# kdavila/lecturemath

Measured on AMD Instinct MI355X. Metric: frames/sec end-to-end binarize+CC+group @1080p, higher is better.
Workload: dtype u8

## Files before the change

lecturemath_amd/csrc/lm_api.hip:

```cpp
#include "lm_common.h"
#include "lm_stream.h"

#include <stdarg.h>
#include <stdlib.h>
#include <stdio.h>
#include <string.h>

#include "../../include/lecturemath_amd.h"

#include "lm_cc_kernels.hip"
#include "lm_match_kernels.hip"
#include "lm_match_batch.hip"
#include "lm_group.hip"
#include "lm_fcn.hip"
#include "lm_fcn2.hip"

static thread_local char g_err[512] = "";

void lm_set_error(const char* fmt, ...)
{
    va_list ap;
    va_start(ap, fmt);
    vsnprintf(g_err, sizeof(g_err), fmt, ap);
    va_end(ap);
// ... 492 lines not shown
    bool ok = hipMemcpy(c->stage_i32, labels, px * sizeof(int32_t), hipMemcpyHostToDevice) == hipSuccess;
    if (ok && ages) ok = hipMemcpy(c->stage_f32, ages, px * sizeof(float), hipMemcpyHostToDevice) == hipSuccess;
    if (ok) {
        const float* d_ages = ages ? c->stage_f32 : (const float*)nullptr;
        hipLaunchKernelGGL(lm_k_ab_init, dim3(lm_blocks(n, 256)), dim3(256), 0, (hipStream_t)0, mny, mxy, mnx, mxx, cnt, ageb, last_px, last_neg,
                           width, height, n);
        hipLaunchKernelGGL(lm_k_ab_scan, dim3(lm_blocks((long long)px, 256)), dim3(256), 0, (hipStream_t)0, c->stage_i32, d_ages, width, height, n,
                           mny, mxy, mnx, mxx, cnt, last_px, last_neg);
        hipLaunchKernelGGL(lm_k_ab_age, dim3(lm_blocks((long long)px, 256)), dim3(256), 0, (hipStream_t)0, c->stage_i32, d_ages, width, height, n,
                           last_neg, ageb);
        hipLaunchKernelGGL(lm_k_ab_finish, dim3(lm_blocks(n, 256)), dim3(256), 0, (hipStream_t)0, ageb, last_px, last_neg, d_ages, agef, n);
        const size_t nb = (size_t)n * sizeof(int32_t);
        ok = hipMemcpy(out_mins_y, mny, nb, hipMemcpyDeviceToHost) == hipSuccess &&
             hipMemcpy(out_maxs_y, mxy, nb, hipMemcpyDeviceToHost) == hipSuccess &&
             hipMemcpy(out_mins_x, mnx, nb, hipMemcpyDeviceToHost) == hipSuccess &&
             hipMemcpy(out_maxs_x, mxx, nb, hipMemcpyDeviceToHost) == hipSuccess &&
             hipMemcpy(out_counts, cnt, nb, hipMemcpyDeviceToHost) == hipSuccess &&
             hipMemcpy(output_age, agef, nb, hipMemcpyDeviceToHost) == hipSuccess;
    }
    if (!ok) lm_set_error("CC_AgeBoundaries: device copy/launch failed");
    (void)hipFree(d_out);
    return 0;
}

extern "C" void lm_stream_destroy(LmStream* s)
{
    if (!s) return;
    void* ptrs[] = {s->cc, s->assign, s->frame_cc_off, s->crop, s->chash, s->active_cc, s->active_box, s->active_last, s->active, s->counters, s->best,
                    s->batch_cc_base, s->batch_word_base};
    for (void* p : ptrs)
        if (p) (void)hipFree(p);
    if (s->mb) {
        LmMatchBatch* m = s->mb;
        void* mp[] = {m->nt_cnt, m->nt_src, m->tlast, m->tcur[0], m->tcur[1], m->ftile_all, m->nt_foff, m->nt_list, m->cls, m->troot, m->rootpos, m->ftile, m->s_prefix, m->tcount[0], m->tcount[1], m->toff[0], m->toff[1], m->pairs[0], m->pairs[1], m->pair_u[0],
                      m->pair_u[1], m->sidx, m->s_list, m->s_box, m->newpos, m->n_src, m->ttab, m->tkey, m->twin, m->big[0], m->big[1], m->n_big};
        for (void* p : mp)
            if (p) (void)hipFree(p);
        delete m;
    }
    if (s->twin_stream) (void)hipStreamDestroy((hipStream_t)s->twin_stream);
    for (int i = 0; i < s->n_run_events; i++) (void)hipEventDestroy(s->run_events[i]);
    free(s->run_events);
    if (s->rd_scratch) (void)hipFree(s->rd_scratch);
    if (s->garena) (void)hipFree(s->garena);
    if (s->gpin) (void)hipHostFree(s->gpin);
    delete s;
}

extern "C" int lm_stream_set_min_pixels(LmStream* s, int min_pixels)
{
    if (!s || min_pixels < 0) { lm_set_error("lm_stream_set_min_pixels: bad arguments"); return LM_ERR_ARG; }
    s->min_pixels = min_pixels;
    return LM_OK;
}

extern "C" int lm_stream_reset(LmStream* s, void* stream)
{
    if (!s) { lm_set_error("lm_stream_reset: null stream"); return LM_ERR_ARG; }
    LM_HIP(hipMemsetAsync(s->counters, 0, sizeof(LmCounters), (hipStream_t)stream));
    LM_HIP(hipMemsetAsync(s->best, 0xff, (size_t)s->ctx->g.cap * sizeof(unsigned long long), (hipStream_t)stream));
    LM_HIP(hipMemsetAsync(s->frame_cc_off, 0, sizeof(long long), (hipStream_t)stream));
    LM_HIP(hipMemsetAsync(s->chash, 0, (size_t)s->cap_cc * sizeof(uint32_t), (hipStream_t)stream));
    if (s->mb) LM_HIP(hipMemsetAsync(s->mb->ttab, 0xff, (size_t)LM_MB_TTAB * sizeof(unsigned long long), (hipStream_t)stream));
    s->frames_pushed = 0;
    s->frames_matched = 0;
    s->tempo_B = 0;
    return LM_OK;
// ... 6 lines not shown
        lm_set_error("lm_stream_create: bad arguments");
        return nullptr;
    }
    LmStream* s = new LmStream();
    memset(s, 0, sizeof(*s));
    s->ctx = ctx;
    s->cap_frames = max_frames;
    s->cap_cc = max_ccs;
    s->cap_words = (unsigned long long)max_crop_words;
    s->cap_uniq = max_uniques;
    s->min_recall = min_recall;
    s->min_precision = min_precision;
    s->max_gap = max_gap;
    s->min_pixels = min_pixels;
    int rc = LM_OK;
    rc |= lm_alloc(&s->cc, (size_t)max_ccs);
    rc |= lm_alloc(&s->assign, (size_t)max_ccs);
    rc |= lm_alloc(&s->frame_cc_off, (size_t)max_frames + 1);
    rc |= lm_alloc(&s->crop, (size_t)max_crop_words);
    rc |= lm_alloc(&s->chash, (size_t)max_ccs);
    rc |= lm_alloc(&s->active_cc, (size_t)max_uniques);
    rc |= lm_alloc(&s->active_box, (size_t)max_uniques);
    rc |= lm_alloc(&s->active_last, (size_t)max_uniques);
    rc |= lm_alloc(&s->active, (size_t)max_uniques);
    rc |= lm_alloc(&s->best, (size_t)ctx->g.cap);
    rc |= lm_alloc(&s->counters, (size_t)1);
    rc |= lm_alloc(&s->batch_cc_base, (size_t)ctx->max_batch);
    rc |= lm_alloc(&s->batch_word_base, (size_t)ctx->max_batch);
    {
        LmMatchBatch* m = new LmMatchBatch();
        memset(m, 0, sizeof(*m));
        s->mb = m;
        m->cap_tiles = (int)(max_ccs / LM_MB_TILE) + max_frames + 2;
        long long cp = 16 * (long long)max_ccs;
        if (cp < (1 << 16)) cp = 1 << 16;
        if (cp > (1 << 23)) cp = 1 << 23;
        m->cap_pairs = (uint32_t)cp;
        rc |= lm_alloc(&m->ftile, (size_t)max_frames + 2);
        rc |= lm_alloc(&m->s_prefix, (size_t)max_frames + 2);
        rc |= lm_alloc(&m->ftile_all, (size_t)max_frames + 2);
        rc |= lm_alloc(&m->nt_foff, (size_t)max_frames + 2);
        rc |= lm_alloc(&m->nt_list, (size_t)max_ccs);
        rc |= lm_alloc(&m->cls, (size_t)max_ccs);
        rc |= lm_alloc(&m->troot, (size_t)max_ccs);
        rc |= lm_alloc(&m->rootpos, (size_t)max_ccs);
        rc |= lm_alloc(&m->nt_cnt, (size_t)LM_MB_MAX_FRAMES);
        rc |= lm_alloc(&m->nt_src, (size_t)max_ccs);
        rc |= lm_alloc(&m->tlast, (size_t)max_ccs);
        for (int k = 0; k < 2; k++) {
            rc |= lm_alloc(&m->tcount[k], (size_t)m->cap_tiles + 1);
            rc |= lm_alloc(&m->toff[k], (size_t)m->cap_tiles + 1);
            rc |= lm_alloc(&m->tcur[k], ((size_t)m->cap_tiles + 1) * LM_MB_JY);
            rc |= lm_alloc(&m->pairs[k], (size_t)m->cap_pairs);
            rc |= lm_alloc(&m->pair_u[k], (size_t)m->cap_pairs);
        }
        rc |= lm_alloc(&m->sidx, (size_t)max_ccs);
        rc |= lm_alloc(&m->s_list, (size_t)max_ccs);
        rc |= lm_alloc(&m->s_box, (size_t)max_ccs);
        rc |= lm_alloc(&m->newpos, (size_t)max_ccs);
        rc |= lm_alloc(&m->n_src, (size_t)1);
        rc |= lm_alloc(&m->ttab, (size_t)LM_MB_TTAB);
        rc |= lm_alloc(&m->tkey, (size_t)max_ccs);
        rc |= lm_alloc(&m->twin, (size_t)max_ccs);
        m->cap_big = 1u << 16;
        rc |= lm_alloc(&m->big[0], (size_t)m->cap_big);
        rc |= lm_alloc(&m->big[1], (size_t)m->cap_big);
        rc |= lm_alloc(&m->n_big, (size_t)2);
#if !LM_HIP_EMULATED
        if (rc == LM_OK &&
            hipFuncSetAttribute((const void*)lm_k_mb_resolve, hipFuncAttributeMaxDynamicSharedMemorySize, (int)LM_MB_RESOLVE_SMEM) != hipSuccess)
            rc = LM_ERR_HIP;
#endif
        const char* e = getenv("LM_MATCH_PER_FRAME");
        s->match_per_frame = (e && atoi(e) == 1) ? 1 : 0;
    }
    if (rc == LM_OK && hipMemset(s->mb->twin, 0, (size_t)max_ccs) != hipSuccess) rc = LM_ERR_HIP;
    if (rc == LM_OK) rc = lm_stream_reset(s, nullptr);
    if (rc == LM_OK && hipStreamSynchronize(nullptr) != hipSuccess) rc = LM_ERR_HIP;
    if (rc != LM_OK) {
        lm_stream_destroy(s);
        return nullptr;
    }
    return s;
}

static void lm_launch_match(LmStream* s, int f, hipStream_t st)
{
    hipLaunchKernelGGL(lm_k_match, LM_HIP_EMULATED ? dim3(2, 2) : dim3(16, 64), dim3(256), 0, st, s->cc, s->crop, s->frame_cc_off, f,
                       s->active_box, s->active_last, s->active_cc, s->counters, s->best, s->min_recall, s->min_precision, s->max_gap);
    hipLaunchKernelGGL(lm_k_update, dim3(1), dim3(1024), 0, st, s->cc, s->frame_cc_off, f, s->active, s->active_cc, s->active_box,
                       s->active_last, s->counters, s->assign, s->best, s->max_gap, s->cap_uniq, (f & 15) == 15 ? 1 : 0);
}

static void lm_flush_tempo(LmStream* s, hipStream_t st)
{
    if (s->tempo_B <= 0) return;
    const LmMatchBatch mb = *s->mb;
    hipLaunchKernelGGL(lm_k_mb_tempo, dim3(LM_HIP_EMULATED ? 2 : 1024), dim3(256), 0, st, s->cc, s->frame_cc_off, s->tempo_f0, s->tempo_B, s->active_box,
                       s->active_cc, s->active_last, s->counters, mb, s->max_gap, s->active, s->assign);
    s->tempo_B = 0;
}

static void lm_launch_match_frames(LmStream* s, int f0, int n, hipStream_t st, hipEvent_t ev_pre = nullptr, bool defer_tempo = false,
                                   hipStream_t st_twin = nullptr, hipEvent_t ev_twin = nullptr, hipEvent_t ev_nt = nullptr)
{
    if (!s->match_per_frame) lm_flush_tempo(s, st);
    if (n > LM_MB_MAX_FRAMES) st_twin = nullptr;
    if (s->match_per_frame) {
        for (int i = 0; i < n; i++) lm_launch_match(s, f0 + i, st);
        return;
    }
    const LmMatchBatch mb = *s->mb;
    const dim3 gj(LM_HIP_EMULATED ? 2 : 128, LM_HIP_EMULATED ? 2 : LM_MB_JY), gt(LM_HIP_EMULATED ? 2 : 1024), ge(LM_HIP_EMULATED ? 2 : 2048), gb(LM_HIP_EMULATED ? 2 : 1024);
    for (int done = 0; done < n;) {
        const int B = (n - done < LM_MB_MAX_FRAMES) ? n - done : LM_MB_MAX_FRAMES;
        const int f = f0 + done;
        s->last_match_frames = B;
        const int twins = (s->min_recall <= 1.0 && s->min_precision <= 1.0) ? 1 : 0;
        if (twins) {
            const dim3 gc(LM_HIP_EMULATED ? 2 : 256);
            const hipStream_t tq = st_twin ? st_twin : st;
            hipLaunchKernelGGL(lm_k_mb_twin_insert, gc, dim3(256), 0, tq, s->cc, s->chash, s->frame_cc_off, f, B, s->counters, mb);
            hipLaunchKernelGGL(lm_k_mb_twin_probe, gc, dim3(256), 0, tq, s->cc, s->frame_cc_off, f, B, s->counters, mb, s->max_gap);
            hipLaunchKernelGGL(lm_k_mb_twin_cmp, ge, dim3(256), 0, tq, s->cc, s->crop, s->frame_cc_off, f, B, s->counters, mb);
            hipLaunchKernelGGL(lm_k_mb_twin_final, gc, dim3(256), 0, tq, s->cc, s->frame_cc_off, f, B, s->counters, mb);
            if (st_twin) { (void)hipEventRecord(ev_twin, st_twin); (void)hipStreamWaitEvent(st, ev_twin, 0); }
        }
        hipLaunchKernelGGL(lm_k_mb_nt, dim3(B + 1), dim3(1024), 0, st, s->frame_cc_off, f, B, s->active, s->active_cc, s->active_box, s->active_last,
                           s->counters, mb, s->max_gap, twins);
        if (twins && st_twin) (void)hipEventRecord(ev_nt, st);
        hipLaunchKernelGGL((lm_k_mb_join<0, 0>), gj, dim3(256), 0, st, s->cc, s->frame_cc_off, f, B, s->active_box, s->active_cc, s->counters, mb);
        hipLaunchKernelGGL((lm_k_mb_join<0, 1>), gj, dim3(256), 0, st, s->cc, s->frame_cc_off, f, B, s->active_box, s->active_cc, s->counters, mb);
        hipLaunchKernelGGL((lm_k_mb_eval<0>), ge, dim3(256), 0, st, s->cc, s->crop, s->frame_cc_off, f, B, s->active_last, s->counters, mb,
                           s->min_recall, s->min_precision, s->max_gap);
        hipLaunchKernelGGL((lm_k_mb_eval_big<0>), gb, dim3(256), 0, st, s->cc, s->crop, s->active_last, s->counters, mb, s->min_recall, s->min_precision,
                           s->max_gap);
        hipLaunchKernelGGL(lm_k_mb_sources, dim3(1), dim3(1024), 0, st, s->cc, s->frame_cc_off, f, B, s->counters, mb);
        hipLaunchKernelGGL((lm_k_mb_join<1, 0>), gj, dim3(256), 0, st, s->cc, s->frame_cc_off, f, B, s->active_box, s->active_cc, s->counters, mb);
        hipLaunchKernelGGL((lm_k_mb_join<1, 1>), gj, dim3(256), 0, st, s->cc, s->frame_cc_off, f, B, s->active_box, s->active_cc, s->counters, mb);
        hipLaunchKernelGGL((lm_k_mb_eval<1>), ge, dim3(256), 0, st, s->cc, s->crop, s->frame_cc_off, f, B, s->active_last, s->counters, mb,
                           s->min_recall, s->min_precision, s->max_gap);
        hipLaunchKernelGGL((lm_k_mb_eval_big<1>), gb, dim3(256), 0, st, s->cc, s->crop, s->active_last, s->counters, mb, s->min_recall, s->min_precision,
                           s->max_gap);
        if (ev_pre && done + B >= n) (void)hipEventRecord(ev_pre, st);
        hipLaunchKernelGGL(lm_k_mb_resolve, dim3(1), dim3(LM_MB_RT), LM_MB_RESOLVE_SMEM, st, s->cc, s->frame_cc_off, f, B, s->active, s->active_cc,
                           s->active_box, s->active_last, s->counters, s->assign, mb, s->max_gap, s->cap_uniq);
        if (defer_tempo && done + B >= n) { s->tempo_f0 = f; s->tempo_B = B; }
        else
            hipLaunchKernelGGL(lm_k_mb_tempo, gt, dim3(256), 0, st, s->cc, s->frame_cc_off, f, B, s->active_box, s->active_cc, s->active_last,
                               s->counters, mb, s->max_gap, s->active, s->assign);
        done += B;
    }
}

static int lm_stream_emit_batch(LmStream* s, int B, void* stream)
{
    LmCtx* c = s->ctx;
    const LmGeom g = c->g;
// ... 65 lines not shown
{
    return lm_stream_push_impl(s, d_binary, n_frames, d_labels, 1, stream);
}

extern "C" int lm_stream_push_records(LmStream* s, const uint8_t* d_binary, int n_frames, int32_t* d_labels, void* stream)
{
    return lm_stream_push_impl(s, d_binary, n_frames, d_labels, 0, stream);
}

static int lm_run_events(LmStream* s, int want)
{
    if (want <= s->n_run_events) return LM_OK;
    want += 192;
    hipEvent_t* ev = (hipEvent_t*)realloc(s->run_events, (size_t)want * sizeof(hipEvent_t));
    if (!ev) { lm_set_error("lm_stream_run_logits: out of memory"); return LM_ERR_HIP; }
    s->run_events = ev;
    for (; s->n_run_events < want; s->n_run_events++) LM_HIP(hipEventCreateWithFlags(&s->run_events[s->n_run_events], hipEventDisableTiming));
    return LM_OK;
}

extern "C" int lm_stream_run_logits(LmStream* s, const float* d_logits, int n_frames, int batch, uint8_t* d_binary, int32_t* d_labels, int thr,
                                    int do_match, int schedule, void* stream_wide, void* stream_match)
{
    if (!s || !d_logits || n_frames < 0 || batch <= 0 || batch > s->ctx->max_batch || schedule < 0 || schedule > 1) {
        lm_set_error("lm_stream_run_logits: bad arguments (batch %d, context batch %d, schedule %d)", batch, s ? s->ctx->max_batch : 0, schedule);
        return LM_ERR_ARG;
    }
    if (do_match && s->frames_matched != s->frames_pushed) {
        lm_set_error("lm_stream_run_logits: %d frames pushed without matching; call lm_stream_match first", s->frames_pushed - s->frames_matched);
        return LM_ERR_STATE;
    }
    hipStream_t sw = (hipStream_t)stream_wide, sm = (hipStream_t)stream_match;
    const bool two = do_match && sm != sw;
    const bool gated = two && schedule == 1 && batch <= LM_MB_MAX_FRAMES && !s->match_per_frame;
    const size_t px = (size_t)s->ctx->g.W * s->ctx->g.H;
    const int nb = (n_frames + batch - 1) / batch;
    if (two) { const int rc = lm_run_events(s, 3 * nb + 2 * nb); if (rc) return rc; }
    hipEvent_t* ev = s->run_events;
    hipEvent_t* ev2 = s->run_events + 3 * nb;
    static const int twin_queue = [] { const char* e = getenv("LM_TWIN_QUEUE"); return e ? atoi(e) : 0; }();
    hipStream_t st_twin = nullptr;
    if (two && twin_queue && !s->match_per_frame && batch <= LM_MB_MAX_FRAMES) {
        if (!s->twin_stream) LM_HIP(hipStreamCreateWithFlags((hipStream_t*)&s->twin_stream, hipStreamNonBlocking));
        st_twin = (hipStream_t)s->twin_stream;
    }
    int prev_n = 0;
    static const int run_ahead = [] { const char* e = getenv("LM_RUN_AHEAD"); return (e && atoi(e) > 0) ? atoi(e) : 0; }();
    for (int k = 0, f0 = 0; f0 < n_frames; f0 += batch, k++) {
        const int n = (n_frames - f0 < batch) ? n_frames - f0 : batch;
        if (two && run_ahead > 0 && k >= run_ahead) LM_HIP(hipEventSynchronize(ev[3 * (k - run_ahead) + 1]));
        if (gated && k >= 2) LM_HIP(hipStreamWaitEvent(sw, ev[3 * (k - 2) + 2], 0));
        int rc = lm_label_batch_logits(s->ctx, d_logits + (size_t)f0 * px, n, thr, 1, d_binary, d_labels, stream_wide);
        if (rc) return rc;
        if (gated) LM_HIP(hipEventRecord(ev[3 * k], sw));
        rc = lm_stream_push_labelled(s, n, stream_wide);
        if (rc) return rc;
        if (!do_match) continue;
        if (!two) {
            rc = lm_stream_match(s, n, stream_wide);
            if (rc) return rc;
        } else if (!gated) {
            LM_HIP(hipEventRecord(ev[3 * k + 1], sw));
            LM_HIP(hipStreamWaitEvent(sm, ev[3 * k + 1], 0));
            if (st_twin) {
                LM_HIP(hipStreamWaitEvent(st_twin, ev[3 * k + 1], 0));
                if (k >= 1) LM_HIP(hipStreamWaitEvent(st_twin, ev2[2 * (k - 1) + 1], 0));
                lm_launch_match_frames(s, s->frames_matched, n, sm, nullptr, false, st_twin, ev2[2 * k], ev2[2 * k + 1]);
                s->frames_matched += n;
            } else {
                rc = lm_stream_match(s, n, stream_match);
                if (rc) return rc;
            }
        } else {
            LM_HIP(hipEventRecord(ev[3 * k + 1], sw));
            if (k >= 1) {
                LM_HIP(hipStreamWaitEvent(sm, ev[3 * k], 0));
                lm_launch_match_frames(s, s->frames_matched, prev_n, sm, ev[3 * (k - 1) + 2], true);
                s->frames_matched += prev_n;
            }
        }
        prev_n = n;
    }
    if (gated && nb > 0) {
        LM_HIP(hipStreamWaitEvent(sm, ev[3 * (nb - 1) + 1], 0));
        lm_launch_match_frames(s, s->frames_matched, prev_n, sm, ev[3 * (nb - 1) + 2]);
        s->frames_matched += prev_n;
    }
    lm_flush_tempo(s, sm);
    LM_HIP(hipGetLastError());
    return LM_OK;
}

extern "C" int lm_stream_match(LmStream* s, int n_frames, void* stream)
{
    if (!s || n_frames < 0 || s->frames_matched + n_frames > s->frames_pushed) {
        lm_set_error("lm_stream_match: %d frames requested, %d pushed, %d matched", n_frames, s ? s->frames_pushed : 0, s ? s->frames_matched : 0);
        return LM_ERR_ARG;
    }
    lm_launch_match_frames(s, s->frames_matched, n_frames, (hipStream_t)stream);
    s->frames_matched += n_frames;
    LM_HIP(hipGetLastError());
    return LM_OK;
}
// ... 406 lines not shown
```

lecturemath_amd/csrc/lm_match_batch.hip:

```cpp
#include "lm_stream.h"

#define LM_MB_TILE 64
#define LM_MB_JY 8
#define LM_MB_TTAB (1 << 18)
#ifndef LM_MB_CHUNK
#define LM_MB_CHUNK 1024
#endif
#define LM_MB_MAX_FRAMES 64
#define LM_MB_BIGPAIR 2048
#ifndef LM_MB_CH
#define LM_MB_CH 2048
#endif
#define LM_MB_LA 16384
#define LM_MB_LS 16384
#ifndef LM_MB_PFA
#define LM_MB_PFA 2
#endif
#ifndef LM_MB_PFB
#define LM_MB_PFB 1
#endif
#define LM_MB_RESOLVE_SMEM ((size_t)LM_MB_CH * 8 + (size_t)LM_MB_LA * 4 + (size_t)LM_MB_LS * 4)

struct LmMatchBatch {
    int32_t* ftile;
    int32_t* ftile_all;
    int32_t* nt_foff;
    int32_t* nt_list;
    int32_t* cls;
    int32_t* troot;
    int32_t* rootpos;
    int32_t* nt_cnt;
    int32_t* nt_src;
    int32_t* tlast;
    int32_t* s_prefix;
    uint32_t* tcount[2];
    uint32_t* toff[2];
    uint32_t* tcur[2];
    uint2* pairs[2];
    int32_t* pair_u[2];
    int32_t* sidx;
    int32_t* s_list;
    unsigned long long* s_box;
    int32_t* newpos;
    int32_t* n_src;
    unsigned long long* ttab;
    uint32_t* tkey;
    uint8_t* twin;
    uint32_t* big[2];
    unsigned* n_big;
    uint32_t cap_big;
    uint32_t cap_pairs;
    int cap_tiles;
};

LM_DEV bool lm_mb_alive(int f, int last, int max_gap) { return f <= 1 || (f - 1) - last < max_gap; }

typedef short lm_s16x2 __attribute__((ext_vector_type(2)));
struct alignas(16) lm_u64x2 { unsigned long long x, y; };
LM_DEV unsigned long long lm_box_as_cc(unsigned long long b)
{
    const unsigned x0 = (unsigned)(b & 0xffff), x1 = (unsigned)((b >> 16) & 0xffff), y0 = (unsigned)((b >> 32) & 0xffff), y1 = (unsigned)(b >> 48);
    return (unsigned long long)(x0 | ((0u - x1) << 16)) | ((unsigned long long)(y0 | ((0u - y1) << 16)) << 32);
// ... 30 lines not shown
                keep[k] = 0;
                if (i < nA) {
                    u[k] = active[i]; uc[k] = active_cc[i]; ub[k] = active_box[i]; ul[k] = active_last[i];
                    keep[k] = lm_mb_alive(f0, ul[k], max_gap) ? 1u : 0u;
                }
                mine += keep[k];
            }
            unsigned tot;
            unsigned ex = lm_block_excl_scan<1024>(mine, &tot);
            unsigned o = kept + ex;
#pragma unroll
            for (int k = 0; k < LM_UPD_ITEMS; k++)
                if (keep[k]) { active[o] = u[k]; active_cc[o] = uc[k]; active_box[o] = ub[k]; active_last[o] = ul[k]; o++; }
            kept += tot;
        }
        nA = (int)kept;
    }
    if (threadIdx.x == 0) {
        *mb.n_src = 0;
        cnt->n_active = nA;
    }
}

#define LM_MB_NT_R 4

__global__ void __launch_bounds__(1024) lm_k_mb_nt(const long long* __restrict__ frame_cc_off, int f0, int B, int32_t* __restrict__ active,
                                                   int32_t* __restrict__ active_cc, unsigned long long* __restrict__ active_box,
                                                   int32_t* __restrict__ active_last, LmCounters* __restrict__ cnt, LmMatchBatch mb, int max_gap,
                                                   int twins)
{
    __shared__ unsigned s_tab[LM_MB_NT_R * 16];
    __shared__ unsigned s_tot;
    __shared__ int s_head[6];
    if (cnt->error) return;
    if ((int)blockIdx.x == B) {
        if (threadIdx.x < 2) mb.n_big[threadIdx.x] = 0;
        lm_mb_prologue(frame_cc_off, f0, B, active, active_cc, active_box, active_last, cnt, mb, max_gap);
        return;
    }
    const int b = (int)blockIdx.x;
    const int lane = lm_lane(), wid = (int)(threadIdx.x >> 6);
    if (wid == 0) {
        unsigned n_nt = 0, n_all = 0;
        if (lane < B) {
            n_all = (unsigned)(frame_cc_off[f0 + lane + 1] - frame_cc_off[f0 + lane]);
            n_nt = twins ? (unsigned)mb.nt_cnt[lane] : n_all;
        }
        const unsigned t_nt = (n_nt + LM_MB_TILE - 1) / LM_MB_TILE, t_all = (n_all + LM_MB_TILE - 1) / LM_MB_TILE;
        const unsigned i_nt = lm_wave_incl_scan(n_nt), i_tnt = lm_wave_incl_scan(t_nt), i_tall = lm_wave_incl_scan(t_all);
        if (lane == b) {
            s_head[0] = (int)(i_nt - n_nt); s_head[1] = (int)(i_tnt - t_nt); s_head[2] = (int)i_tnt;
            mb.nt_foff[b] = (int32_t)(i_nt - n_nt);
            mb.ftile[b] = (int32_t)(i_tnt - t_nt);
            mb.ftile_all[b] = (int32_t)(i_tall - t_all);
            if (b == B - 1) {
                mb.nt_foff[B] = (int32_t)i_nt;
                mb.ftile[B] = (int32_t)i_tnt;
                mb.ftile_all[B] = (int32_t)i_tall;
                if ((int)i_tnt > mb.cap_tiles || (int)i_tall > mb.cap_tiles) cnt->error = LM_ERR_CAPACITY;
            }
        }
    }
    __syncthreads();
    const int t0 = s_head[1], t1 = s_head[2] + (b == B - 1 ? 1 : 0);
    for (int t = t0 + (int)threadIdx.x; t < t1 && t <= mb.cap_tiles; t += 1024) { mb.tcount[0][t] = 0; mb.tcount[1][t] = 0; }
    const long long C0 = frame_cc_off[f0 + b], C1 = frame_cc_off[f0 + b + 1];
    unsigned carry = (unsigned)s_head[0];
    for (long long base = C0; base < C1; base += 1024 * LM_MB_NT_R) {
        unsigned fm = 0;
#pragma unroll
        for (int k = 0; k < LM_MB_NT_R; k++) {
            const long long i = base + (long long)k * 1024 + threadIdx.x;
            const int flag = (i < C1) ? (mb.twin[i] == 0) : 0;
            fm |= (unsigned)flag << k;
            const unsigned long long bal = __ballot(flag);
            if (lane == 0) s_tab[k * 16 + wid] = (unsigned)__popcll(bal);
        }
        __syncthreads();
        if (wid == 0) {
            const unsigned v = s_tab[lane];
            const unsigned incl = lm_wave_incl_scan(v);
            s_tab[lane] = incl - v;
            if (lane == 63) s_tot = incl;
        }
        __syncthreads();
#pragma unroll
        for (int k = 0; k < LM_MB_NT_R; k++) {
            const int flag = (int)((fm >> k) & 1u);
            const unsigned long long bal = __ballot(flag);
            const long long i = base + (long long)k * 1024 + threadIdx.x;
            if (flag) {
                const unsigned o = carry + s_tab[k * 16 + wid] + (unsigned)__popcll(bal & lm_lowmask_excl(lane));
                mb.nt_list[o] = (int32_t)i; mb.cls[i] = (int32_t)o; mb.tlast[o] = -1; mb.sidx[i] = -2;
            }
        }
        carry += s_tot;
        __syncthreads();
    }
}

LM_DEV int lm_mb_tile_frame(const int32_t* __restrict__ ftile, int B, int t)
{
    const int lane = lm_lane();
    const unsigned long long le = __ballot(lane < B && ftile[lane] <= t);
    return 63 - __clzll((long long)le);
}

template <int SRC, int FILL>
__global__ void __launch_bounds__(256) lm_k_mb_join(const LmCcRec* __restrict__ cc, const long long* __restrict__ frame_cc_off, int f0,
                                                    int B, const unsigned long long* __restrict__ active_box,
                                                    const int32_t* __restrict__ active_cc, LmCounters* __restrict__ cnt, LmMatchBatch mb)
{
    __shared__ __attribute__((aligned(16))) unsigned long long s_sbox[LM_MB_CHUNK + 4];
    __shared__ int s_spos[LM_MB_CHUNK];
    __shared__ int s_ub[4];
    __shared__ int s_nsurv;
    __shared__ unsigned s_count, s_base;
    if (cnt->error) return;
    const int nt = mb.ftile[B];
    const unsigned long long* src_box = SRC == 0 ? active_box : mb.s_box;
    const int32_t* src_cc = SRC == 0 ? active_cc : mb.s_list;
    const int ccl = (int)(threadIdx.x & 63), q = (int)(threadIdx.x >> 6);
    for (int t = blockIdx.x; t < nt; t += gridDim.x) {
        const int b = lm_mb_tile_frame(mb.ftile, B, t);
        const int n_all = SRC == 0 ? cnt->n_active : mb.s_prefix[b];
        const int s_lo = (int)((long long)n_all * blockIdx.y / gridDim.y), s_hi = (int)((long long)n_all * (blockIdx.y + 1) / gridDim.y);
        const int k_first = mb.nt_foff[b] + (t - mb.ftile[b]) * LM_MB_TILE;
        const int ncc = (mb.nt_foff[b + 1] - k_first < LM_MB_TILE) ? mb.nt_foff[b + 1] - k_first : LM_MB_TILE;
        __syncthreads();
        if (threadIdx.x == 0) { s_ub[0] = 0x7fff; s_ub[1] = -1; s_ub[2] = 0x7fff; s_ub[3] = -1; s_count = 0; }
        unsigned off = 0;
        if (FILL) {
            unsigned part = 0;
            for (int i = threadIdx.x; i < t; i += 256) part += mb.tcount[SRC][i];
            unsigned tot;
            (void)lm_block_excl_scan<256>(part, &tot);
            off = tot;
        }
// ... 149 lines not shown
            if (SRC == 0 && lm_mb_alive(rec.frame, active_last[pr.y], max_gap)) mb.sidx[ci] = -1;
        }
    }
}

template <int SRC>
__global__ void __launch_bounds__(256) lm_k_mb_eval_big(const LmCcRec* __restrict__ cc, const uint32_t* __restrict__ crop,
                                                        const int32_t* __restrict__ active_last, LmCounters* __restrict__ cnt, LmMatchBatch mb,
                                                        double min_recall, double min_precision, int max_gap)
{
    __shared__ int s_sum;
    if (cnt->error) return;
    const unsigned n = mb.n_big[SRC] < mb.cap_big ? mb.n_big[SRC] : mb.cap_big;
    for (unsigned b = blockIdx.x; b < n; b += gridDim.x) {
        const unsigned p = mb.big[SRC][b];
        const uint2 pr = mb.pairs[SRC][p];
        const long long ci = (long long)mb.nt_list[pr.x];
        const LmCcRec rec = cc[ci], urec = cc[mb.pair_u[SRC][p]];
        const LmIsect is = lm_isect(rec, urec);
        if (threadIdx.x == 0) s_sum = 0;
        __syncthreads();
        int m = lm_overlap_words(rec, urec, is, crop, (int)threadIdx.x, 256);
        m = lm_wave_sum(m);
        if (lm_lane() == 0 && m) atomicAdd(&s_sum, m);
        __syncthreads();
        if (threadIdx.x == 0 && lm_accept(s_sum, rec.size, urec.size, min_recall, min_precision)) {
            mb.pairs[SRC][p].x = pr.x | 0x80000000u;
            if (SRC == 0 && lm_mb_alive(rec.frame, active_last[pr.y], max_gap)) mb.sidx[ci] = -1;
        }
        __syncthreads();
    }
}

__global__ void __launch_bounds__(256) lm_k_mb_twin_insert(const LmCcRec* __restrict__ cc, const uint32_t* __restrict__ chash,
                                                           const long long* __restrict__ frame_cc_off, int f0, int B,
                                                           LmCounters* __restrict__ cnt, LmMatchBatch mb)
{
    if (cnt->error) return;
    const long long C0 = frame_cc_off[f0], C1 = frame_cc_off[f0 + B];
    const long long n = C1 - C0;
    if (blockIdx.x == 0 && threadIdx.x < LM_MB_MAX_FRAMES) mb.nt_cnt[threadIdx.x] = 0;
    if (n * 2 > LM_MB_TTAB) return;
    for (long long i = (long long)blockIdx.x * blockDim.x + threadIdx.x; i < n; i += (long long)gridDim.x * blockDim.x) {
        const LmCcRec r = cc[C0 + i];
        const unsigned h = chash[C0 + i];
        const unsigned long long box = lm_pack_box(r);
        unsigned key = lm_mix32(h ^ lm_mix32((unsigned)box) ^ lm_mix32((unsigned)(box >> 32) + 0x85ebca6bu) ^ lm_mix32((unsigned)r.size + 0xc2b2ae35u));
        if (key == 0xffffffffu) key = 0;
        mb.tkey[C0 + i] = key;
        const unsigned long long val = ((unsigned long long)key << 32) | (unsigned long long)(unsigned)i;
        for (unsigned probe = 0; probe < LM_MB_TTAB; probe++) {
            const unsigned slot = (key + probe) & (LM_MB_TTAB - 1);
            const unsigned long long old = atomicCAS(&mb.ttab[slot], ~0ull, val);
            if (old == ~0ull) break;
            if ((unsigned)(old >> 32) == key) { atomicMin(&mb.ttab[slot], val); break; }
        }
    }
}

__global__ void __launch_bounds__(256) lm_k_mb_twin_probe(const LmCcRec* __restrict__ cc, const long long* __restrict__ frame_cc_off, int f0, int B,
                                                          LmCounters* __restrict__ cnt, LmMatchBatch mb, int max_gap)
{
    if (cnt->error) return;
    const long long C0 = frame_cc_off[f0], C1 = frame_cc_off[f0 + B];
    const long long n = C1 - C0;
    const bool enabled = n * 2 <= LM_MB_TTAB;
    for (long long i = (long long)blockIdx.x * blockDim.x + threadIdx.x; i < n; i += (long long)gridDim.x * blockDim.x) {
        long long root = -1;
        if (enabled) {
            const unsigned key = mb.tkey[C0 + i];
            for (unsigned probe = 0; probe < LM_MB_TTAB; probe++) {
                const unsigned slot = (key + probe) & (LM_MB_TTAB - 1);
                const unsigned long long e = mb.ttab[slot];
                if (e == ~0ull) break;
                if ((unsigned)(e >> 32) == key) {
                    root = (long long)(unsigned)e;
                    mb.tkey[C0 + i] = slot;
                    break;
                }
            }
            if (root >= 0 && root < i) {
                const LmCcRec r = cc[C0 + i], q = cc[C0 + root];
                if (!(r.size == q.size && r.min_x == q.min_x && r.max_x == q.max_x && r.min_y == q.min_y && r.max_y == q.max_y &&
                      q.frame < r.frame && r.frame - q.frame <= max_gap))
                    root = -1;
            } else {
                root = -1;
            }
        }
        mb.twin[C0 + i] = root >= 0 ? 1 : 0;
        mb.troot[C0 + i] = root >= 0 ? (int32_t)(C0 + root) : -1;
    }
}

LM_DEV long long lm_cc_of_word(const LmCcRec* __restrict__ cc, long long C0, long long n, unsigned long long w, long long start)
{
    long long k = start;
    while (k + 1 < n && cc[C0 + k + 1].crop_off <= w) k++;
    return k;
}

LM_DEV long long lm_cc_of_word_search(const LmCcRec* __restrict__ cc, long long C0, long long n, unsigned long long w)
{
    long long lo = 0, hi = n;
    while (hi - lo > 1) {
        const long long mid = (lo + hi) >> 1;
        if (cc[C0 + mid].crop_off <= w) lo = mid; else hi = mid;
    }
    return lo;
}

#define LM_TW_WIN 256
#define LM_TW_UNR 4

__global__ void __launch_bounds__(256) lm_k_mb_twin_cmp(const LmCcRec* __restrict__ cc, const uint32_t* __restrict__ crop,
                                                        const long long* __restrict__ frame_cc_off, int f0, int B,
                                                        LmCounters* __restrict__ cnt, LmMatchBatch mb)
{
    __shared__ unsigned long long s_off[LM_TW_WIN + 1], s_roff[LM_TW_WIN];
    __shared__ int s_root[LM_TW_WIN];
    __shared__ int s_cnt4[4], s_any;
    if (cnt->error) return;
    const long long C0 = frame_cc_off[f0], C1 = frame_cc_off[f0 + B];
    const long long n = C1 - C0;
    if (n <= 0 || n * 2 > LM_MB_TTAB) return;
    const unsigned long long W0 = cc[C0].crop_off;
    const LmCcRec last = cc[C1 - 1];
    const unsigned long long W1 = last.crop_off + (unsigned long long)((last.max_x >> 5) - (last.min_x >> 5) + 1) *
                                                      (unsigned long long)(last.max_y - last.min_y + 1);
    constexpr unsigned long long STEP = 256ull * LM_TW_UNR;
    const unsigned long long per = (((W1 - W0 + gridDim.x - 1) / gridDim.x + STEP - 1) / STEP) * STEP;
    const unsigned long long wb0 = W0 + (unsigned long long)blockIdx.x * per;
    if (wb0 >= W1) return;
    const unsigned long long wb1 = (W1 - wb0 < per) ? W1 : wb0 + per;
    const int tid = (int)threadIdx.x, lane = lm_lane();
    long long klo = 0;
    for (long long len = n; len > 1;) {
        const long long stride = (len + 255) >> 8;
        const bool in = (long long)tid * stride < len;
        const unsigned long long bal = __ballot(in && cc[C0 + klo + tid * stride].crop_off <= wb0);
        __syncthreads();
        if (lane == 0) s_cnt4[tid >> 6] = (int)__popcll(bal);
        __syncthreads();
        const int c = s_cnt4[0] + s_cnt4[1] + s_cnt4[2] + s_cnt4[3];
        klo += (c - 1) * stride;
        len = (len - (c - 1) * stride < stride) ? len - (c - 1) * stride : stride;
    }
    for (unsigned long long cur = wb0; cur < wb1;) {
        const int nwin = (n - klo < LM_TW_WIN) ? (int)(n - klo) : LM_TW_WIN;
        __syncthreads();
        if (tid == 0) s_any = 0;
        __syncthreads();
        if (tid < nwin) {
            const int32_t root = mb.troot[C0 + klo + tid];
            s_off[tid] = cc[C0 + klo + tid].crop_off;
            s_root[tid] = root;
            s_roff[tid] = root >= 0 ? cc[root].crop_off : 0ull;
            if (root >= 0) s_any = 1;
        }
        if (tid == 0) s_off[nwin] = (klo + nwin < n) ? cc[C0 + klo + nwin].crop_off : W1;
        __syncthreads();
        const unsigned long long wend = s_off[nwin] < wb1 ? s_off[nwin] : wb1;
        if (s_any) {
            for (unsigned long long w0 = cur + (unsigned long long)(tid & ~63) * LM_TW_UNR; w0 < wend; w0 += STEP) {
                int jj[LM_TW_UNR];
                unsigned mine[LM_TW_UNR], theirs[LM_TW_UNR];
#pragma unroll
                for (int u = 0; u < LM_TW_UNR; u++) {
                    const unsigned long long w = w0 + (unsigned long long)(u * 64 + lane);
                    jj[u] = -1; mine[u] = 0; theirs[u] = 0;
                    if (w < wend) {
                        int lo = 0, hi = nwin;
                        while (hi - lo > 1) {
                            const int mid = (lo + hi) >> 1;
                            if (s_off[mid] <= w) lo = mid; else hi = mid;
                        }
                        if (s_root[lo] >= 0) {
                            jj[u] = lo;
                            mine[u] = crop[w];
                            theirs[u] = crop[s_roff[lo] + (w - s_off[lo])];
                        }
                    }
                }
#pragma unroll
                for (int u = 0; u < LM_TW_UNR; u++)
                    if (jj[u] >= 0 && mine[u] != theirs[u]) mb.twin[C0 + klo + jj[u]] = 0;
            }
        }
        cur = wend;
        klo += nwin;
    }
}

__global__ void __launch_bounds__(256) lm_k_mb_twin_final(const LmCcRec* __restrict__ cc, const long long* __restrict__ frame_cc_off, int f0, int B,
                                                          LmCounters* __restrict__ cnt, LmMatchBatch mb)
{
    if (cnt->error) return;
    const long long C0 = frame_cc_off[f0], C1 = frame_cc_off[f0 + B];
    const int lane = lm_lane();
    if ((C1 - C0) * 2 <= LM_MB_TTAB)
        for (long long i = C0 + (long long)blockIdx.x * blockDim.x + threadIdx.x; i < C1; i += (long long)gridDim.x * blockDim.x)
            mb.ttab[mb.tkey[i] & (LM_MB_TTAB - 1)] = ~0ull;
    for (long long base = C0 + ((long long)blockIdx.x * blockDim.x + (threadIdx.x & ~63u)); base < C1; base += (long long)gridDim.x * blockDim.x) {
        const long long i = base + lane;
        const bool nt = i < C1 && !mb.twin[i];
        int fb = -1;
        if (nt) { mb.troot[i] = -1; fb = cc[i].frame - f0; }
        unsigned long long todo = __ballot(nt);
        while (todo) {
            const int leader = __ffsll((long long)todo) - 1;
            const int fl = __shfl(fb, leader);
            const unsigned long long same = __ballot(nt && fb == fl);
            if (lane == leader) atomicAdd(&mb.nt_cnt[fl], (int)__popcll(same));
            todo &= ~same;
        }
    }
}

__global__ void __launch_bounds__(256) lm_k_crop_hash(const LmCcRec* __restrict__ cc, const uint32_t* __restrict__ crop, long long c0, long long n,
                                                      unsigned long long W1, uint32_t* __restrict__ chash)
{
    if (n <= 0) return;
    const unsigned long long W0 = cc[c0].crop_off;
    const int lane = lm_lane();
    const unsigned long long wave = ((unsigned long long)blockIdx.x * blockDim.x + threadIdx.x) >> 6, nwaves = ((unsigned long long)gridDim.x * blockDim.x) >> 6;
    for (unsigned long long w0 = W0 + wave * 64ull; w0 < W1; w0 += nwaves * 64ull) {
        const long long k0 = lm_cc_of_word_search(cc, c0, n, w0);
        const unsigned long long w = w0 + (unsigned long long)lane;
        const bool live = w < W1;
        long long k = k0;
        unsigned contrib = 0;
        if (live) {
            k = lm_cc_of_word(cc, c0, n, w, k0);
            contrib = lm_mix32(crop[w] + 0x9e3779b9u * (unsigned)(w - cc[c0 + k].crop_off));
        }
        const bool same = live && k == k0;
        const unsigned wsum = lm_wave_sum(same ? contrib : 0u);
        if (lane == 0 && live) atomicAdd(&chash[c0 + k0], wsum);
        if (live && !same) atomicAdd(&chash[c0 + k], contrib);
    }
// ... 388 lines not shown
```

lecturemath_amd/csrc/lm_stream.h:

```cpp
#pragma once
#include "lm_common.h"

struct __attribute__((aligned(32))) LmCcRec {
    int32_t cc_id;
    int32_t size;
    int16_t min_x, max_x, min_y, max_y;
    unsigned long long crop_off;
    int32_t frame;
    int32_t pad;
};

struct LmCounters {
    long long n_cc;
    unsigned long long n_words;
    unsigned long long tempo_count;
    int n_frames;
    int n_matched;
    int n_uniq;
    int n_active;
    int error;
    int pad;
};

struct LmStream {
    LmCtx* ctx;
    long long cap_cc;
    unsigned long long cap_words;
    int cap_frames, cap_uniq;
    double min_recall, min_precision;
    int max_gap, min_pixels;
    LmCcRec* cc;
    int32_t* assign;
    long long* frame_cc_off;
    uint32_t* crop;
    uint32_t* chash;
    int32_t* active;
    int32_t* active_cc;
    unsigned long long* active_box;
    int32_t* active_last;
    unsigned long long* best;
    LmCounters* counters;
    long long* batch_cc_base;
    unsigned long long* batch_word_base;
    void* rd_scratch;
    size_t rd_scratch_bytes;
    void* garena;
    size_t garena_bytes;
    int garena_busy;
    void* gpin;
    size_t gpin_bytes;
    int gpin_busy;
    struct LmMatchBatch* mb;
    int last_match_frames;
    int match_per_frame;
    hipEvent_t* run_events;
    int n_run_events;
    void* twin_stream;
    int tempo_f0, tempo_B;
    int frames_pushed;
    int frames_matched;
};
```

Measured before the change: 72710.

## Widen batched matching window with bucketed twin chains and deferred match launches

Raises the max frames per batched match from 64 to 256 and adds a configurable match window. Matching is deferred until a full window of frames is pending, so fewer, larger match batches are launched. Twin detection now hashes per 64-frame bucket and links roots across buckets with a new chain-resolution kernel. The cost is larger buffers (pairs, hash table, big lists), an extra kernel, multi-wave scans per frame, and longer latency before frames are matched.

```diff
diff --git a/lecturemath_amd/csrc/lm_api.hip b/lecturemath_amd/csrc/lm_api.hip
--- a/lecturemath_amd/csrc/lm_api.hip
+++ b/lecturemath_amd/csrc/lm_api.hip
@@ -548,7 +548,7 @@
         if (p) (void)hipFree(p);
     if (s->mb) {
         LmMatchBatch* m = s->mb;
-        void* mp[] = {m->nt_cnt, m->nt_src, m->tlast, m->tcur[0], m->tcur[1], m->ftile_all, m->nt_foff, m->nt_list, m->cls, m->troot, m->rootpos, m->ftile, m->s_prefix, m->tcount[0], m->tcount[1], m->toff[0], m->toff[1], m->pairs[0], m->pairs[1], m->pair_u[0],
+        void* mp[] = {m->nt_cnt, m->nt_src, m->tlast, m->tcur[0], m->tcur[1], m->ftile_all, m->tpar, m->tcand, m->glast, m->nt_foff, m->nt_list, m->cls, m->troot, m->rootpos, m->ftile, m->s_prefix, m->tcount[0], m->tcount[1], m->toff[0], m->toff[1], m->pairs[0], m->pairs[1], m->pair_u[0],
                       m->pair_u[1], m->sidx, m->s_list, m->s_box, m->newpos, m->n_src, m->ttab, m->tkey, m->twin, m->big[0], m->big[1], m->n_big};
         for (void* p : mp)
             if (p) (void)hipFree(p);
@@ -621,9 +621,9 @@
         memset(m, 0, sizeof(*m));
         s->mb = m;
         m->cap_tiles = (int)(max_ccs / LM_MB_TILE) + max_frames + 2;
-        long long cp = 16 * (long long)max_ccs;
-        if (cp < (1 << 16)) cp = 1 << 16;
-        if (cp > (1 << 23)) cp = 1 << 23;
+        long long cp = 64 * (long long)max_ccs;
+        if (cp < (1 << 20)) cp = 1 << 20;
+        if (cp > (1 << 24)) cp = 1 << 24;
         m->cap_pairs = (uint32_t)cp;
         rc |= lm_alloc(&m->ftile, (size_t)max_frames + 2);
         rc |= lm_alloc(&m->s_prefix, (size_t)max_frames + 2);
@@ -632,6 +632,9 @@
         rc |= lm_alloc(&m->nt_list, (size_t)max_ccs);
         rc |= lm_alloc(&m->cls, (size_t)max_ccs);
         rc |= lm_alloc(&m->troot, (size_t)max_ccs);
+        rc |= lm_alloc(&m->tpar, (size_t)max_ccs);
+        rc |= lm_alloc(&m->tcand, (size_t)max_ccs);
+        rc |= lm_alloc(&m->glast, (size_t)max_ccs);
         rc |= lm_alloc(&m->rootpos, (size_t)max_ccs);
         rc |= lm_alloc(&m->nt_cnt, (size_t)LM_MB_MAX_FRAMES);
         rc |= lm_alloc(&m->nt_src, (size_t)max_ccs);
@@ -651,7 +654,7 @@
         rc |= lm_alloc(&m->ttab, (size_t)LM_MB_TTAB);
         rc |= lm_alloc(&m->tkey, (size_t)max_ccs);
         rc |= lm_alloc(&m->twin, (size_t)max_ccs);
-        m->cap_big = 1u << 16;
+        m->cap_big = 1u << 18;
         rc |= lm_alloc(&m->big[0], (size_t)m->cap_big);
         rc |= lm_alloc(&m->big[1], (size_t)m->cap_big);
         rc |= lm_alloc(&m->n_big, (size_t)2);
@@ -662,6 +665,9 @@
 #endif
         const char* e = getenv("LM_MATCH_PER_FRAME");
         s->match_per_frame = (e && atoi(e) == 1) ? 1 : 0;
+        e = getenv("LM_MATCH_WINDOW");
+        const int wdef = max_gap < 64 ? 64 : (max_gap > LM_MB_MAX_FRAMES ? LM_MB_MAX_FRAMES : max_gap);
+        s->match_window = (e && atoi(e) >= 1 && atoi(e) <= LM_MB_MAX_FRAMES) ? atoi(e) : wdef;
     }
     if (rc == LM_OK && hipMemset(s->mb->twin, 0, (size_t)max_ccs) != hipSuccess) rc = LM_ERR_HIP;
     if (rc == LM_OK) rc = lm_stream_reset(s, nullptr);
@@ -694,7 +700,7 @@
                                    hipStream_t st_twin = nullptr, hipEvent_t ev_twin = nullptr, hipEvent_t ev_nt = nullptr)
 {
     if (!s->match_per_frame) lm_flush_tempo(s, st);
-    if (n > LM_MB_MAX_FRAMES) st_twin = nullptr;
+    if (n > s->match_window) st_twin = nullptr;
     if (s->match_per_frame) {
         for (int i = 0; i < n; i++) lm_launch_match(s, f0 + i, st);
         return;
@@ -702,7 +708,7 @@
     const LmMatchBatch mb = *s->mb;
     const dim3 gj(LM_HIP_EMULATED ? 2 : 128, LM_HIP_EMULATED ? 2 : LM_MB_JY), gt(LM_HIP_EMULATED ? 2 : 1024), ge(LM_HIP_EMULATED ? 2 : 2048), gb(LM_HIP_EMULATED ? 2 : 1024);
     for (int done = 0; done < n;) {
-        const int B = (n - done < LM_MB_MAX_FRAMES) ? n - done : LM_MB_MAX_FRAMES;
+        const int B = (n - done < s->match_window) ? n - done : s->match_window;
         const int f = f0 + done;
         s->last_match_frames = B;
         const int twins = (s->min_recall <= 1.0 && s->min_precision <= 1.0) ? 1 : 0;
@@ -713,6 +719,7 @@
             hipLaunchKernelGGL(lm_k_mb_twin_probe, gc, dim3(256), 0, tq, s->cc, s->frame_cc_off, f, B, s->counters, mb, s->max_gap);
             hipLaunchKernelGGL(lm_k_mb_twin_cmp, ge, dim3(256), 0, tq, s->cc, s->crop, s->frame_cc_off, f, B, s->counters, mb);
             hipLaunchKernelGGL(lm_k_mb_twin_final, gc, dim3(256), 0, tq, s->cc, s->frame_cc_off, f, B, s->counters, mb);
+            hipLaunchKernelGGL(lm_k_mb_twin_chain, gc, dim3(256), 0, tq, s->cc, s->frame_cc_off, f, B, s->counters, mb, s->max_gap);
             if (st_twin) { (void)hipEventRecord(ev_twin, st_twin); (void)hipStreamWaitEvent(st, ev_twin, 0); }
         }
         hipLaunchKernelGGL(lm_k_mb_nt, dim3(B + 1), dim3(1024), 0, st, s->frame_cc_off, f, B, s->active, s->active_cc, s->active_box, s->active_last,
@@ -844,7 +851,7 @@
     }
     hipStream_t sw = (hipStream_t)stream_wide, sm = (hipStream_t)stream_match;
     const bool two = do_match && sm != sw;
-    const bool gated = two && schedule == 1 && batch <= LM_MB_MAX_FRAMES && !s->match_per_frame;
+    const bool gated = two && schedule == 1 && batch <= s->match_window && !s->match_per_frame;
     const size_t px = (size_t)s->ctx->g.W * s->ctx->g.H;
     const int nb = (n_frames + batch - 1) / batch;
     if (two) { const int rc = lm_run_events(s, 3 * nb + 2 * nb); if (rc) return rc; }
@@ -852,7 +859,7 @@
     hipEvent_t* ev2 = s->run_events + 3 * nb;
     static const int twin_queue = [] { const char* e = getenv("LM_TWIN_QUEUE"); return e ? atoi(e) : 0; }();
     hipStream_t st_twin = nullptr;
-    if (two && twin_queue && !s->match_per_frame && batch <= LM_MB_MAX_FRAMES) {
+    if (two && twin_queue && !s->match_per_frame && batch <= s->match_window) {
         if (!s->twin_stream) LM_HIP(hipStreamCreateWithFlags((hipStream_t*)&s->twin_stream, hipStreamNonBlocking));
         st_twin = (hipStream_t)s->twin_stream;
     }
@@ -873,14 +880,18 @@
             if (rc) return rc;
         } else if (!gated) {
             LM_HIP(hipEventRecord(ev[3 * k + 1], sw));
-            LM_HIP(hipStreamWaitEvent(sm, ev[3 * k + 1], 0));
+            const int pending = s->frames_pushed - s->frames_matched;
+            const bool tail = f0 + n >= n_frames;
             if (st_twin) {
+                LM_HIP(hipStreamWaitEvent(sm, ev[3 * k + 1], 0));
                 LM_HIP(hipStreamWaitEvent(st_twin, ev[3 * k + 1], 0));
                 if (k >= 1) LM_HIP(hipStreamWaitEvent(st_twin, ev2[2 * (k - 1) + 1], 0));
                 lm_launch_match_frames(s, s->frames_matched, n, sm, nullptr, false, st_twin, ev2[2 * k], ev2[2 * k + 1]);
                 s->frames_matched += n;
-            } else {
-                rc = lm_stream_match(s, n, stream_match);
+            } else if (s->match_per_frame || tail || pending >= s->match_window) {
+                LM_HIP(hipStreamWaitEvent(sm, ev[3 * k + 1], 0));
+                const int m = (s->match_per_frame || tail) ? pending : pending - pending % s->match_window;
+                rc = lm_stream_match(s, m, stream_match);
                 if (rc) return rc;
             }
         } else {
diff --git a/lecturemath_amd/csrc/lm_match_batch.hip b/lecturemath_amd/csrc/lm_match_batch.hip
--- a/lecturemath_amd/csrc/lm_match_batch.hip
+++ b/lecturemath_amd/csrc/lm_match_batch.hip
@@ -2,11 +2,15 @@
 
 #define LM_MB_TILE 64
 #define LM_MB_JY 8
-#define LM_MB_TTAB (1 << 18)
+#define LM_MB_TTAB (1 << 20)
 #ifndef LM_MB_CHUNK
 #define LM_MB_CHUNK 1024
 #endif
-#define LM_MB_MAX_FRAMES 64
+#ifndef LM_MB_MAX_FRAMES
+#define LM_MB_MAX_FRAMES 256
+#endif
+#define LM_MB_TBUCKET 64
+static_assert(LM_MB_MAX_FRAMES % 64 == 0 && LM_MB_MAX_FRAMES <= 1024, "per-frame scans: one thread per frame, whole waves");
 #define LM_MB_BIGPAIR 2048
 #ifndef LM_MB_CH
 #define LM_MB_CH 2048
@@ -28,6 +32,9 @@
     int32_t* nt_list;
     int32_t* cls;
     int32_t* troot;
+    int32_t* tpar;
+    uint8_t* tcand;
+    int32_t* glast;
     int32_t* rootpos;
     int32_t* nt_cnt;
     int32_t* nt_src;
@@ -124,6 +131,7 @@
     __shared__ unsigned s_tab[LM_MB_NT_R * 16];
     __shared__ unsigned s_tot;
     __shared__ int s_head[6];
+    __shared__ unsigned s_wt[LM_MB_MAX_FRAMES / 64][3];
     if (cnt->error) return;
     if ((int)blockIdx.x == B) {
         if (threadIdx.x < 2) mb.n_big[threadIdx.x] = 0;
@@ -132,15 +140,19 @@
     }
     const int b = (int)blockIdx.x;
     const int lane = lm_lane(), wid = (int)(threadIdx.x >> 6);
-    if (wid == 0) {
+    {
+        const int fb = (int)threadIdx.x;
         unsigned n_nt = 0, n_all = 0;
-        if (lane < B) {
-            n_all = (unsigned)(frame_cc_off[f0 + lane + 1] - frame_cc_off[f0 + lane]);
-            n_nt = twins ? (unsigned)mb.nt_cnt[lane] : n_all;
+        if (fb < B) {
+            n_all = (unsigned)(frame_cc_off[f0 + fb + 1] - frame_cc_off[f0 + fb]);
+            n_nt = twins ? (unsigned)mb.nt_cnt[fb] : n_all;
         }
         const unsigned t_nt = (n_nt + LM_MB_TILE - 1) / LM_MB_TILE, t_all = (n_all + LM_MB_TILE - 1) / LM_MB_TILE;
-        const unsigned i_nt = lm_wave_incl_scan(n_nt), i_tnt = lm_wave_incl_scan(t_nt), i_tall = lm_wave_incl_scan(t_all);
-        if (lane == b) {
+        unsigned i_nt = lm_wave_incl_scan(n_nt), i_tnt = lm_wave_incl_scan(t_nt), i_tall = lm_wave_incl_scan(t_all);
+        if (wid < LM_MB_MAX_FRAMES / 64 && lane == 63) { s_wt[wid][0] = i_nt; s_wt[wid][1] = i_tnt; s_wt[wid][2] = i_tall; }
+        __syncthreads();
+        if (fb == b) {
+            for (int w = 0; w < wid; w++) { i_nt += s_wt[w][0]; i_tnt += s_wt[w][1]; i_tall += s_wt[w][2]; }
             s_head[0] = (int)(i_nt - n_nt); s_head[1] = (int)(i_tnt - t_nt); s_head[2] = (int)i_tnt;
             mb.nt_foff[b] = (int32_t)(i_nt - n_nt);
             mb.ftile[b] = (int32_t)(i_tnt - t_nt);
@@ -194,8 +206,13 @@
 LM_DEV int lm_mb_tile_frame(const int32_t* __restrict__ ftile, int B, int t)
 {
     const int lane = lm_lane();
-    const unsigned long long le = __ballot(lane < B && ftile[lane] <= t);
-    return 63 - __clzll((long long)le);
+    int le[LM_MB_MAX_FRAMES / 64];
+#pragma unroll
+    for (int c = 0; c < LM_MB_MAX_FRAMES / 64; c++) le[c] = (c * 64 + lane < B) ? ftile[c * 64 + lane] : 0x7fffffff;
+    int n = 0;
+#pragma unroll
+    for (int c = 0; c < LM_MB_MAX_FRAMES / 64; c++) n += (int)__popcll(__ballot(le[c] <= t));
+    return n - 1;
 }
 
 template <int SRC, int FILL>
@@ -411,6 +428,26 @@
     }
 }
 
+LM_DEV unsigned lm_mb_tkey(unsigned key, int bucket)
+{
+    unsigned k = lm_mix32(key ^ (0x9e3779b9u * (unsigned)(bucket + 1)));
+    return k == 0xffffffffu ? 0u : k;
+}
+
+LM_DEV long long lm_mb_tfind(const unsigned long long* __restrict__ ttab, unsigned key, unsigned* slot_out)
+{
+    for (unsigned probe = 0; probe < LM_MB_TTAB; probe++) {
+        const unsigned slot = (key + probe) & (LM_MB_TTAB - 1);
+        const unsigned long long e = ttab[slot];
+        if (e == ~0ull) return -1;
+        if ((unsigned)(e >> 32) == key) {
+            if (slot_out) *slot_out = slot;
+            return (long long)(unsigned)e;
+        }
+    }
+    return -1;
+}
+
 __global__ void __launch_bounds__(256) lm_k_mb_twin_insert(const LmCcRec* __restrict__ cc, const uint32_t* __restrict__ chash,
                                                            const long long* __restrict__ frame_cc_off, int f0, int B,
                                                            LmCounters* __restrict__ cnt, LmMatchBatch mb)
@@ -418,21 +455,22 @@
     if (cnt->error) return;
     const long long C0 = frame_cc_off[f0], C1 = frame_cc_off[f0 + B];
     const long long n = C1 - C0;
-    if (blockIdx.x == 0 && threadIdx.x < LM_MB_MAX_FRAMES) mb.nt_cnt[threadIdx.x] = 0;
+    if (blockIdx.x == 0)
+        for (int k = (int)threadIdx.x; k < LM_MB_MAX_FRAMES; k += (int)blockDim.x) mb.nt_cnt[k] = 0;
     if (n * 2 > LM_MB_TTAB) return;
     for (long long i = (long long)blockIdx.x * blockDim.x + threadIdx.x; i < n; i += (long long)gridDim.x * blockDim.x) {
         const LmCcRec r = cc[C0 + i];
         const unsigned h = chash[C0 + i];
         const unsigned long long box = lm_pack_box(r);
-        unsigned key = lm_mix32(h ^ lm_mix32((unsigned)box) ^ lm_mix32((unsigned)(box >> 32) + 0x85ebca6bu) ^ lm_mix32((unsigned)r.size + 0xc2b2ae35u));
-        if (key == 0xffffffffu) key = 0;
+        const unsigned key = lm_mix32(h ^ lm_mix32((unsigned)box) ^ lm_mix32((unsigned)(box >> 32) + 0x85ebca6bu) ^ lm_mix32((unsigned)r.size + 0xc2b2ae35u));
         mb.tkey[C0 + i] = key;
-        const unsigned long long val = ((unsigned long long)key << 32) | (unsigned long long)(unsigned)i;
+        const unsigned bkey = lm_mb_tkey(key, (r.frame - f0) / LM_MB_TBUCKET);
+        const unsigned long long val = ((unsigned long long)bkey << 32) | (unsigned long long)(unsigned)i;
         for (unsigned probe = 0; probe < LM_MB_TTAB; probe++) {
-            const unsigned slot = (key + probe) & (LM_MB_TTAB - 1);
+            const unsigned slot = (bkey + probe) & (LM_MB_TTAB - 1);
             const unsigned long long old = atomicCAS(&mb.ttab[slot], ~0ull, val);
             if (old == ~0ull) break;
-            if ((unsigned)(old >> 32) == key) { atomicMin(&mb.ttab[slot], val); break; }
+            if ((unsigned)(old >> 32) == bkey) { atomicMin(&mb.ttab[slot], val); break; }
         }
     }
 }
@@ -445,30 +483,35 @@
     const long long n = C1 - C0;
     const bool enabled = n * 2 <= LM_MB_TTAB;
     for (long long i = (long long)blockIdx.x * blockDim.x + threadIdx.x; i < n; i += (long long)gridDim.x * blockDim.x) {
-        long long root = -1;
+        long long par = -1;
+        int cand = 0;
+        const LmCcRec r = cc[C0 + i];
         if (enabled) {
             const unsigned key = mb.tkey[C0 + i];
-            for (unsigned probe = 0; probe < LM_MB_TTAB; probe++) {
-                const unsigned slot = (key + probe) & (LM_MB_TTAB - 1);
-                const unsigned long long e = mb.ttab[slot];
-                if (e == ~0ull) break;
-                if ((unsigned)(e >> 32) == key) {
-                    root = (long long)(unsigned)e;
-                    mb.tkey[C0 + i] = slot;
-                    break;
-                }
-            }
+            const int bk = (r.frame - f0) / LM_MB_TBUCKET;
+            unsigned slot = 0;
+            const long long root = lm_mb_tfind(mb.ttab, lm_mb_tkey(key, bk), &slot);
+            mb.tkey[C0 + i] = slot;
             if (root >= 0 && root < i) {
-                const LmCcRec r = cc[C0 + i], q = cc[C0 + root];
-                if (!(r.size == q.size && r.min_x == q.min_x && r.max_x == q.max_x && r.min_y == q.min_y && r.max_y == q.max_y &&
-                      q.frame < r.frame && r.frame - q.frame <= max_gap))
-                    root = -1;
-            } else {
-                root = -1;
-            }
-        }
-        mb.twin[C0 + i] = root >= 0 ? 1 : 0;
-        mb.troot[C0 + i] = root >= 0 ? (int32_t)(C0 + root) : -1;
+                const LmCcRec q = cc[C0 + root];
+                if (r.size == q.size && r.min_x == q.min_x && r.max_x == q.max_x && r.min_y == q.min_y && r.max_y == q.max_y &&
+                    q.frame < r.frame && r.frame - q.frame <= max_gap && (q.frame - f0) / LM_MB_TBUCKET == bk) {
+                    par = root; cand = 1;
+                }
+            } else if (root == i && bk > 0) {
+                const long long p = lm_mb_tfind(mb.ttab, lm_mb_tkey(key, bk - 1), nullptr);
+                if (p >= 0) {
+                    const LmCcRec q = cc[C0 + p];
+                    if (r.size == q.size && r.min_x == q.min_x && r.max_x == q.max_x && r.min_y == q.min_y && r.max_y == q.max_y &&
+                        (q.frame - f0) / LM_MB_TBUCKET == bk - 1) {
+                        par = p; cand = 2;
+                    }
+                }
+            }
+        }
+        mb.tcand[C0 + i] = (uint8_t)cand;
+        mb.tpar[C0 + i] = par >= 0 ? (int32_t)(C0 + par) : -1;
+        mb.glast[C0 + i] = r.frame;
     }
 }
 
@@ -531,7 +574,7 @@
         if (tid == 0) s_any = 0;
         __syncthreads();
         if (tid < nwin) {
-            const int32_t root = mb.troot[C0 + klo + tid];
+            const int32_t root = mb.tpar[C0 + klo + tid];
             s_off[tid] = cc[C0 + klo + tid].crop_off;
             s_root[tid] = root;
             s_roff[tid] = root >= 0 ? cc[root].crop_off : 0ull;
@@ -563,7 +606,7 @@
                 }
 #pragma unroll
                 for (int u = 0; u < LM_TW_UNR; u++)
-                    if (jj[u] >= 0 && mine[u] != theirs[u]) mb.twin[C0 + klo + jj[u]] = 0;
+                    if (jj[u] >= 0 && mine[u] != theirs[u]) mb.tcand[C0 + klo + jj[u]] = 0;
             }
         }
         cur = wend;
@@ -576,15 +619,37 @@
 {
     if (cnt->error) return;
     const long long C0 = frame_cc_off[f0], C1 = frame_cc_off[f0 + B];
+    if ((C1 - C0) * 2 <= LM_MB_TTAB)
+        for (long long i = C0 + (long long)blockIdx.x * blockDim.x + threadIdx.x; i < C1; i += (long long)gridDim.x * blockDim.x) {
+            mb.ttab[mb.tkey[i] & (LM_MB_TTAB - 1)] = ~0ull;
+            if (mb.tcand[i] == 1) atomicMax(&mb.glast[mb.tpar[i]], cc[i].frame);
+        }
+}
+
+__global__ void __launch_bounds__(256) lm_k_mb_twin_chain(const LmCcRec* __restrict__ cc, const long long* __restrict__ frame_cc_off, int f0, int B,
+                                                          LmCounters* __restrict__ cnt, LmMatchBatch mb, int max_gap)
+{
+    if (cnt->error) return;
+    const long long C0 = frame_cc_off[f0], C1 = frame_cc_off[f0 + B];
     const int lane = lm_lane();
-    if ((C1 - C0) * 2 <= LM_MB_TTAB)
-        for (long long i = C0 + (long long)blockIdx.x * blockDim.x + threadIdx.x; i < C1; i += (long long)gridDim.x * blockDim.x)
-            mb.ttab[mb.tkey[i] & (LM_MB_TTAB - 1)] = ~0ull;
     for (long long base = C0 + ((long long)blockIdx.x * blockDim.x + (threadIdx.x & ~63u)); base < C1; base += (long long)gridDim.x * blockDim.x) {
         const long long i = base + lane;
-        const bool nt = i < C1 && !mb.twin[i];
+        bool nt = false;
         int fb = -1;
-        if (nt) { mb.troot[i] = -1; fb = cc[i].frame - f0; }
+        if (i < C1) {
+            long long node = i;
+            for (;;) {
+                const int c = mb.tcand[node];
+                if (c == 0) break;
+                const long long p = mb.tpar[node];
+                if (c == 2 && cc[node].frame - mb.glast[p] > max_gap) break;
+                node = p;
+            }
+            nt = node == i;
+            mb.twin[i] = nt ? 0 : 1;
+            mb.troot[i] = nt ? -1 : (int32_t)node;
+            if (nt) fb = cc[i].frame - f0;
+        }
         unsigned long long todo = __ballot(nt);
         while (todo) {
             const int leader = __ffsll((long long)todo) - 1;
diff --git a/lecturemath_amd/csrc/lm_stream.h b/lecturemath_amd/csrc/lm_stream.h
--- a/lecturemath_amd/csrc/lm_stream.h
+++ b/lecturemath_amd/csrc/lm_stream.h
@@ -53,6 +53,7 @@
     struct LmMatchBatch* mb;
     int last_match_frames;
     int match_per_frame;
+    int match_window;
     hipEvent_t* run_events;
     int n_run_events;
     void* twin_stream;
```

Result: faster. 76890, median of 6 (+5.7%).
